# RomanJuranek/librectify

Hardware: AMD Instinct MI355X
Metric: Mpix/s end-to-end (detect+VP) on 4K frames, batch call of 64 frames, 5 in flight (higher is better)
Workload: dtype f32

## Files before the change

librectify_amd/csrc/common.h:

```cpp
#pragma once
#include <hip/hip_runtime.h>

#include <cstdint>
#include <string>

#include "../../include/librectify_amd.h"

namespace lramd {

constexpr float kEps = 1e-6f;
constexpr int kMaxModels = 4;
constexpr int kMaxPeelModels = 5;
constexpr float kInlierDeg = 2.0f;
constexpr float kGarbageDeg = 4.0f;
constexpr int kRansacMaxIter = 10000;
constexpr int kEdgeKernelSize = 2;
constexpr float kEdgeKernelSigma = 1.0f;
constexpr int kSeedDist = 2;
constexpr float kSeedRatio = 0.95f;
constexpr float kTraceTolerance = 0.25f;
constexpr float kLineMaxErr = 2.0f;
constexpr float kLineMinLength = 5.f;
constexpr int kComponentMinSize = 5;
constexpr int kBins = 8;
// ... 138 lines not shown
    BinTrig trig;
    uint32_t* label;
    int32_t* seed_size;
    int32_t* queue;
    const uint4* seed_rec;
};
struct FloodProgress {
    int enqueued = 0;
    bool use_big = false;
    int win_growth = 2;
    bool sizes_known = false;
    uint32_t max_flood = 0;
};
constexpr int kFloodCtrlWords = 56;
int flood_enqueue(const FloodBuffers& B, const FloodFrame& F, FloodProgress* P, uint32_t* h_ctrl, hipStream_t s);
int flood_finish(const FloodBuffers& B, const FloodFrame& F, FloodProgress* P, uint32_t* h_ctrl, int* rounds_out,
                 uint32_t* tiers_out ,
                 bool* extra, hipStream_t s);

size_t fit_temp_bytes(size_t max_pixels, uint32_t max_segments);
struct HugeSort {
    uint32_t* tab = nullptr;
    uint32_t* list = nullptr;
    uint32_t* jobs = nullptr;
    uint32_t max = 0;
};
int launch_component_offsets(const int32_t* seed_size, const uint32_t* d_n_seeds, uint32_t seed_cap, int min_size,
                             uint32_t* comp_rank, uint32_t* comp_seed, uint32_t* comp_off,
                             uint32_t* totals , uint32_t* large_list, uint32_t large_cap,
                             uint32_t* n_large, void* temp, size_t temp_bytes, uint32_t frame_tag, uint32_t* cursor, const HugeSort& hs,
                             hipStream_t s);
int launch_component_scatter(const uint32_t* label, size_t npix, const uint32_t* comp_rank, const uint32_t* comp_off,
                             uint32_t* cursor, uint32_t* px, const HugeSort& hs, uint32_t* n_large, bool with_huge, hipStream_t s);
int launch_component_sort(const uint32_t* px_in, uint32_t* px_out, const uint32_t* comp_off, const uint32_t* d_n_comp,
                          uint32_t comp_cap, const uint32_t* large_list, uint32_t large_cap, const uint32_t* n_large,
                          uint32_t* scratch, const uint32_t* cursor, const HugeSort& hs, bool with_huge, hipStream_t s);
int launch_fit(const uint32_t* px_sorted, const uint32_t* px_unsorted, const uint32_t* comp_off, const uint32_t* comp_seed, const uint32_t* d_n_comp,
               uint32_t comp_cap, const int32_t* seed_bin, const float* dx, const float* dy, int w, BinTrig trig,
               float* scratch_w, LineSegment* out, const uint32_t* cursor, const HugeSort& hs, const uint32_t* n_large, bool with_huge,
               hipStream_t s);

struct PencilSoA {
    const float* ax;
    const float* ay;
    const float* dx;
    const float* dy;
    const float* len;
    const float* hx;
    const float* hy;
    const float* hz;
};
constexpr int kRansacBestSlots = 32;
int launch_ransac_score(PencilSoA m, uint32_t n, float tol, float degeneracy_tol, uint32_t n_iter, uint64_t seed,
                        uint32_t round, unsigned long long* best_slots, uint32_t* host_best, hipStream_t s);
int launch_ransac_score_dev(PencilSoA m, const uint32_t* gctl, int max_models, float tol, float degeneracy_tol,
                            uint32_t n_iter, uint64_t seed, unsigned long long* best_slots, hipStream_t s);

struct PencilTable {
    float* ax;
    float* ay;
    float* dx;
    float* dy;
    float* len;
    float* hx;
    float* hy;
    float* hz;
    uint32_t* orig;
    PencilSoA soa() const { return PencilSoA{ax, ay, dx, dy, len, hx, hy, hz}; }
};
enum {
    kGcLines = 0,
    kGcRemaining = 1,
    kGcRound = 2,
// ... 30 lines not shown
```

librectify_amd/csrc/frame.hip:

```cpp
#include "host.h"

#include <cstdio>
#include <cstdlib>
#include <cstring>

namespace lramd {


namespace {

uint32_t round_up(uint32_t v, uint32_t m) { return (v + m - 1) / m * m; }

uint32_t initial_seed_cap(size_t npix) {
    return (uint32_t)std::min<size_t>(npix, std::max<size_t>(round_up((uint32_t)(npix / 32), 1024), 4096));
}

uint32_t line_cap_for(const lr_context* c) {
    return (uint32_t)std::min<size_t>(c->seed_cap, c->ws.cap_pix / 6 + 16);
}


PencilTable table_of(lr_context* c, int which) {
    const size_t cl = c->cap_glines;
    float* b = c->d_tables + (size_t)which * 8 * cl;
// ... 151 lines not shown
}

int finish_flood(lr_context* c, bool* extra) {
    *extra = false;
    if (c->opt.flood_mode == 0) return 0;
    if (flood_finish(flood_buffers_for(c), flood_frame_for(c), &c->flood_prog, c->h_counts + 16, &c->flood_rounds,
                     c->flood_tiers, extra, c->stream))
        return 1;
    static const bool call_debug = std::getenv("LIBRECTIFY_CALL_DEBUG") != nullptr;
    if (call_debug)
        std::fprintf(stderr, "flood: %d rounds, %u walks in the second tier, %u of them long, hold-back phase %u (started with it: %d)\n",
                     c->flood_rounds, c->flood_tiers[0], c->flood_tiers[8], c->flood_tiers[3], (int)c->flood_hold_hint);
    c->flood_logbig_hint = c->flood_tiers[0] > 0;
    c->flood_calm_hint = c->flood_tiers[0] == 0 && c->flood_tiers[1] == 0 && c->flood_tiers[15] == 0;
    c->flood_big_hint = true;
    c->flood_hold_hint = c->flood_tiers[3] != 0 && c->flood_tiers[8] >= 16;
    constexpr uint32_t kStagedKeep = 64;
    c->flood_staged_hint = c->flood_tiers[14] != 0 && (!c->flood_staged_hint || c->flood_tiers[0] >= kStagedKeep);
    c->flood_staged_streak = c->flood_staged_hint ? c->flood_staged_streak + 1 : 0;
    if (c->flood_staged_streak >= 16) {
        c->flood_staged_hint = false;
        c->flood_staged_streak = 0;
    }
    if (c->flood_staged_hint) c->flood_hold_hint = false;

    c->flood_rounds_hint = std::max(std::max(c->flood_rounds + 2, 6), c->flood_rounds_hint - 1);
    c->flood_rounds_last = c->flood_rounds;
    return 0;
}

int enqueue_fit(lr_context* c) {
    const size_t npix = (size_t)c->w * c->h;
    const uint32_t comp_cap = line_cap_for(c);
    const bool with_huge = !(c->opt.flood_mode != 0 && c->flood_prog.sizes_known && c->flood_prog.max_flood <= (1u << 14));
    if (launch_component_offsets(c->ws.seed_size, c->d_counts + kCntSeeds, c->seed_cap, kComponentMinSize, c->ws.comp_rank,
                                 c->ws.comp_seed, c->ws.comp_off, c->d_counts + kCntComp, c->ws.comp_large,
                                 (uint32_t)(c->ws.cap_pix / 64 + 16), c->d_counts + kCntLarge, c->ws.temp, c->ws.temp.cap(), ++c->fit_tag ? c->fit_tag : ++c->fit_tag, c->ws.cursor,
                                 with_huge ? c->ws.huge : HugeSort{}, c->stream))
        return 1;
    if (launch_component_scatter(c->ws.label, npix, c->ws.comp_rank, c->ws.comp_off, c->ws.cursor, c->ws.px_a, c->ws.huge, c->d_counts + kCntLarge, with_huge,
                                 c->stream))
        return 1;
    if (launch_component_sort(c->ws.px_a, c->ws.px_b, c->ws.comp_off, c->d_counts + kCntComp, comp_cap, c->ws.comp_large,
                              (uint32_t)(c->ws.cap_pix / 64 + 16), c->d_counts + kCntLarge, reinterpret_cast<uint32_t*>(c->ws.keys_b.get()),
                              c->ws.cursor, c->ws.huge, with_huge, c->stream))
        return 1;
    static const bool fit_debug = std::getenv("LIBRECTIFY_FIT_DEBUG") != nullptr;
    if (fit_debug) {
        uint32_t cnt[16];
        LR_HIP(hipStreamSynchronize(c->stream));
        LR_HIP(hipMemcpy(cnt, c->d_counts, sizeof(cnt), hipMemcpyDeviceToHost));
        std::fprintf(stderr, "fit: with_huge %d (sizes known %d, largest flood %u); seeds %u comps %u px %u; lists: %u of 65..1024 px, %u longer, %u huge in %u buckets; counter %u\n",
                     (int)with_huge, (int)c->flood_prog.sizes_known, c->flood_prog.max_flood, cnt[0], cnt[1], cnt[2], cnt[4], cnt[5], cnt[6], cnt[7], cnt[10]);
        const uint32_t nj = std::min<uint32_t>(cnt[7], 6);
        std::vector<uint32_t> jobs(4 * nj + 4);
        if (nj) LR_HIP(hipMemcpy(jobs.data(), c->ws.huge.jobs, nj * 16, hipMemcpyDeviceToHost));
        for (uint32_t j = 0; j < nj; ++j) std::fprintf(stderr, "   bucket job %u: start %u, %u px, table word %u\n", j, jobs[4 * j], jobs[4 * j + 1], jobs[4 * j + 2]);
    }
    if (launch_fit(c->ws.px_b, c->ws.px_a, c->ws.comp_off, c->ws.comp_seed, c->d_counts + kCntComp, comp_cap, c->ws.seed_bin, c->ws.dx, c->ws.dy, c->w,
                   c->trig, c->ws.scratch_w, c->ws.d_lines, c->ws.cursor, c->ws.huge, c->d_counts + kCntLarge, with_huge, c->stream))
        return 1;
    if (c->opt.timing_on) LR_HIP(hipEventRecord(c->ev[4], c->stream));
    return 0;
}

}

int enqueue_groups(lr_context* c, uint32_t line_cap, int max_models, float inlier_deg, float garbage_deg, int n_iter,
                   uint64_t seed, bool model_done, bool gather) {
    if (max_models > kMaxPeelModels) {
        set_error("estimate_line_pencils: max_models above " + std::to_string(kMaxPeelModels) + " (the reference uses 4, config.h:25)");
        return 1;
    }
    const float tol = cos_threshold(inlier_deg), garbage_tol = cos_threshold(garbage_deg);
    const PencilTable all = table_of(c, 0);
    PencilTable tab[2] = {table_of(c, 1), table_of(c, 2)};
    if (!model_done && launch_pencil_model(c->d_flines, c->d_gctl, c->d_gnorm, all, tab[0], line_cap, c->stream)) return 1;
    const float degeneracy_tol = 0.05f;
    for (int k = 0; k < max_models; ++k) {
        if (n_iter > 0 &&
            launch_ransac_score_dev(tab[k & 1].soa(), c->d_gctl, max_models, tol, degeneracy_tol, (uint32_t)n_iter, seed,
                                    c->d_best_slots, c->stream))
            return 1;
        const bool last = gather && k == max_models - 1;
        if (launch_peel(tab[k & 1], tab[(k + 1) & 1], all, c->d_best_slots, seed, tol, garbage_tol,
                        max_models, c->d_gctl, c->d_inl, c->d_flines, c->d_models, c->d_counts,
                        (uint32_t)std::min<size_t>(c->res_lines_cap, c->d_flines.cap()), last ? c->h_res.get() : nullptr, c->stream))
            return 1;
    }
    return 0;
}

namespace {
// ... 374 lines not shown
```

librectify_amd/csrc/kernels_fit.hip:

```cpp
#include <algorithm>
#include <cstring>

#include <atomic>

#include "common.h"

namespace lramd {
namespace {

constexpr uint32_t kNoComp = 0xFFFFFFFFu;

constexpr uint32_t kSortLds = 1024;
constexpr uint32_t kSortLdsBig = 16384;
constexpr uint32_t kHugeShift = 14;
constexpr uint32_t kHugeFlag = 0x80000000u;
constexpr int kOffPer = 8;
constexpr uint32_t kOffChunk = 256 * kOffPer;

__device__ __forceinline__ void chunk_counts(const int32_t* __restrict__ seed_size, uint32_t n_seeds, int min_size,
                                             uint32_t k0, int (&sz)[kOffPer], uint32_t& c, uint32_t& p) {
    c = p = 0;
#pragma unroll
    for (int j = 0; j < kOffPer; ++j) {
        sz[j] = (k0 + j < n_seeds) ? seed_size[k0 + j] : 0;
// ... 178 lines not shown
    if (nn > 0.0) {
        vr = vr / nn;
        vc = vc / nn;
    } else {
        vr = 1.0;
        vc = 0.0;
    }
    float fr = (float)vr, fc = (float)vc;
    if (fr < fc || (fr == fc && fr < 0.0f)) {
        fr = -fr;
        fc = -fc;
    }
    d_r = fr;
    d_c = fc;
}

template <int kThreads, class Keys>
__device__ __forceinline__ void bitonic_sort(Keys& key, uint32_t P) {
    for (uint32_t k = 2; k <= P; k <<= 1)
        for (uint32_t j = k >> 1; j > 0; j >>= 1) {
            for (uint32_t t = threadIdx.x; t < P / 2; t += kThreads) {
                const uint32_t i = 2 * t - (t & (j - 1));
                const uint32_t a = key[i], b = key[i + j];
                const bool up = (i & k) == 0;
                if ((a > b) == up) {
                    key[i] = b;
                    key[i + j] = a;
                }
            }
            __syncthreads();
        }
}

__global__ __launch_bounds__(256) void component_sort_large_kernel(const uint32_t* __restrict__ px_in,
                                                                   uint32_t* __restrict__ px_out,
                                                                   const uint32_t* __restrict__ comp_off,
                                                                   const uint32_t* __restrict__ large_list,
                                                                   const uint32_t* __restrict__ n_large) {
    __shared__ uint32_t s_key[kSortLds];
    const uint32_t n_list = n_large[0];
    for (uint32_t li = blockIdx.x; li < n_list; li += gridDim.x) {
        const uint32_t comp = large_list[li];
        const uint32_t off = comp_off[comp];
        const uint32_t n = comp_off[comp + 1] - off;
        uint32_t P = 128;
        while (P < n) P <<= 1;
        for (uint32_t i = threadIdx.x; i < P; i += 256) s_key[i] = i < n ? px_in[off + i] : 0xFFFFFFFFu;
        __syncthreads();
        bitonic_sort<256>(s_key, P);
        for (uint32_t i = threadIdx.x; i < n; i += 256) px_out[off + i] = s_key[i];
        __syncthreads();
    }
}

template <bool kGlobal>
__global__ __launch_bounds__(1024) void component_sort_big_kernel(const uint32_t* __restrict__ px_in,
                                                                  uint32_t* __restrict__ px_out,
                                                                  const uint32_t* __restrict__ comp_off,
                                                                  const uint32_t* __restrict__ large_list,
                                                                  uint32_t large_cap,
                                                                  const uint32_t* __restrict__ n_large,
                                                                  uint32_t* __restrict__ scratch,
                                                                  const uint32_t* __restrict__ cursor) {
    __shared__ uint32_t s_key[kGlobal ? 1 : kSortLdsBig];
    const uint32_t n_list = n_large[1];
    for (uint32_t li = blockIdx.x; li < n_list; li += gridDim.x) {
        const uint32_t comp = large_list[large_cap - 1u - li];
        const uint32_t off = comp_off[comp];
        const uint32_t n = comp_off[comp + 1] - off;
        if ((n > kSortLdsBig) != kGlobal) continue;
        if (kGlobal && cursor != nullptr && (cursor[comp] & kHugeFlag)) continue;
        uint32_t P = 2048;
        while (P < n) P <<= 1;
        if (!kGlobal) {
            for (uint32_t i = threadIdx.x; i < P; i += 1024) s_key[i] = i < n ? px_in[off + i] : 0xFFFFFFFFu;
            __syncthreads();
            bitonic_sort<1024>(s_key, P);
            for (uint32_t i = threadIdx.x; i < n; i += 1024) px_out[off + i] = s_key[i];
            __syncthreads();
        } else {
            for (uint32_t i = threadIdx.x; i < P; i += 1024) scratch[i] = i < n ? px_in[off + i] : 0xFFFFFFFFu;
            __syncthreads();
            bitonic_sort<1024>(scratch, P);
            for (uint32_t i = threadIdx.x; i < n; i += 1024) px_out[off + i] = scratch[i];
            __syncthreads();
        }
    }
}

__global__ __launch_bounds__(256) void huge_count_kernel(const uint32_t* __restrict__ label, size_t npix,
                                                         const uint32_t* __restrict__ comp_rank,
                                                         const uint32_t* __restrict__ comp_off,
                                                         const uint32_t* __restrict__ cursor, uint32_t* __restrict__ huge_tab,
                                                         uint32_t nb, const uint32_t* __restrict__ huge_list, uint32_t huge_max,
                                                         uint4* __restrict__ jobs, uint32_t* __restrict__ n_large) {
    const uint32_t n_huge = min(n_large[2], huge_max);
    if (n_huge == 0u) return;
    const int lane = threadIdx.x & 63;
    const size_t step = (size_t)gridDim.x * 256;
    const size_t n_pad = (npix + 255) / 256 * 256;
    for (size_t i = (size_t)blockIdx.x * 256 + threadIdx.x; i < n_pad; i += step) {
        const uint32_t l = i < npix ? label[i] : kLabelFree;
        const uint32_t r = l != kLabelFree ? comp_rank[l] : kNoComp;
        uint32_t hi = 0u;
        if (r != kNoComp && comp_off[r + 1u] - comp_off[r] > kSortLdsBig) hi = cursor[r];
        uint64_t todo = __ballot((hi & kHugeFlag) != 0u);
        while (todo != 0ull) {
            const int leader = __builtin_ctzll(todo);
            const uint32_t hl = (uint32_t)__builtin_amdgcn_readlane((int)hi, leader);
            const uint64_t same = __ballot(hi == hl) & todo;
            if (lane == leader) atomicAdd(&huge_tab[(size_t)(hl & ~kHugeFlag) * nb + (uint32_t)(i >> kHugeShift)], (uint32_t)__popcll(same));
            todo &= ~same;
        }
    }
    __shared__ uint32_t s_last;
    __syncthreads();
    if (threadIdx.x == 0) {
        __threadfence();
        s_last = atomicAdd(n_large + 6, 1u) == gridDim.x - 1u ? 1u : 0u;
// ... 14 lines not shown
            for (int off = 1; off < 64; off <<= 1) {
                const uint32_t t = (uint32_t)__shfl_up((int)inc, off);
                if (lane >= off) inc += t;
            }
            const uint32_t start = run + inc - cnt;
            if (cnt != 0u) {
                *e = start;
                jobs[atomicAdd(n_large + 3, 1u)] = make_uint4(start, cnt, h * nb + b, 0u);
            }
            run += (uint32_t)__shfl((int)inc, 63);
        }
    }
}

__global__ __launch_bounds__(1024) void huge_sort_kernel(const uint32_t* __restrict__ px_in, uint32_t* __restrict__ px_out,
                                                         const uint4* __restrict__ jobs, uint32_t* __restrict__ huge_tab,
                                                         const uint32_t* __restrict__ n_large) {
    __shared__ uint32_t s_key[kSortLdsBig];
    const uint32_t n_jobs = n_large[3];
    for (uint32_t j = blockIdx.x; j < n_jobs; j += gridDim.x) {
        const uint4 job = jobs[j];
        const uint32_t off = job.x, n = job.y;
        uint32_t P = 64;
        while (P < n) P <<= 1;
        for (uint32_t i = threadIdx.x; i < P; i += 1024) s_key[i] = i < n ? px_in[off + i] : 0xFFFFFFFFu;
        __syncthreads();
        bitonic_sort<1024>(s_key, P);
        for (uint32_t i = threadIdx.x; i < n; i += 1024) px_out[off + i] = s_key[i];
        if (threadIdx.x == 0) huge_tab[job.z] = 0u;
        __syncthreads();
    }
}

template <int kU>
__device__ __forceinline__ void fit_large(const uint32_t* __restrict__ px, uint32_t comp, uint32_t off, uint32_t n, float s, float c,
                                          uint32_t uw, const float* __restrict__ dx, const float* __restrict__ dy,
                                          float* __restrict__ scratch_w, LineSegment* __restrict__ out, int lane) {
    float acc = 0.f;
    for (uint32_t i0 = lane; i0 < n; i0 += 64u * kU) {
        uint32_t p[kU];
        float gx[kU], gy[kU];
#pragma unroll
        for (int u = 0; u < kU; ++u) {
            const uint32_t i = i0 + 64u * (uint32_t)u;
            p[u] = i < n ? px[off + i] : 0u;
        }
#pragma unroll
        for (int u = 0; u < kU; ++u) {
            gx[u] = dx[p[u]];
            gy[u] = dy[p[u]];
        }
#pragma unroll
        for (int u = 0; u < kU; ++u) {
            const uint32_t i = i0 + 64u * (uint32_t)u;
            if (i < n) {
                const float wv = directional(gx[u], gy[u], s, c);
                scratch_w[off + i] = wv;
                acc = acc + wv;
            }
        }
    }
    const float S = wave_tree(acc);

    float ar = 0.f, ac = 0.f;
    for (uint32_t i0 = lane; i0 < n; i0 += 64u * kU) {
        uint32_t p[kU];
// ... 42 lines not shown
    }
    const float cov_rr = wave_tree(crr), cov_rc = wave_tree(crc), cov_cc = wave_tree(ccc);

    float d_r, d_c;
    major_axis_2x2(cov_rr, cov_rc, cov_cc, d_r, d_c);
    const float n_r = -d_c, n_c = d_r;

    float t0 = INFINITY, t1 = -INFINITY, es = 0.f;
    for (uint32_t i0 = lane; i0 < n; i0 += 64u * kU) {
        uint32_t p[kU];
#pragma unroll
        for (int u = 0; u < kU; ++u) {
            const uint32_t i = i0 + 64u * (uint32_t)u;
            p[u] = i < n ? px[off + i] : 0u;
        }
#pragma unroll
        for (int u = 0; u < kU; ++u) {
            const uint32_t i = i0 + 64u * (uint32_t)u;
            if (i < n) {
                const float cr = (float)(p[u] / uw) - a_r, cc = (float)(p[u] % uw) - a_c;
                const float t = cr * d_r + cc * d_c;
                t0 = fminf(t0, t);
                t1 = fmaxf(t1, t);
                es = es + fabsf(cr * n_r + cc * n_c);
            }
        }
    }
#pragma unroll
    for (int o = 32; o >= 1; o >>= 1) {
        t0 = fminf(t0, __shfl_xor(t0, o));
        t1 = fmaxf(t1, __shfl_xor(t1, o));
    }
    const float esum = wave_tree(es);
    if (lane == 0) {
        LineSegment l;
        l.x1 = a_c + d_c * t0;
        l.y1 = a_r + d_r * t0;
        l.x2 = a_c + d_c * t1;
        l.y2 = a_r + d_r * t1;
        l.weight = S / (float)n;
        l.err = esum / (float)n;
        l.group_id = -1;
        out[comp] = l;
    }
}

__global__ __launch_bounds__(256) void fit_kernel(const uint32_t* __restrict__ px, const uint32_t* __restrict__ px_unsorted,
                                                  const uint32_t* __restrict__ comp_off,
                                                  const uint32_t* __restrict__ comp_seed, const uint32_t* __restrict__ n_comp_ptr,
                                                  const int32_t* __restrict__ seed_bin, const float* __restrict__ dx,
                                                  const float* __restrict__ dy, int w, BinTrig trig,
                                                  float* __restrict__ scratch_w, LineSegment* __restrict__ out,
                                                  const uint32_t* __restrict__ huge_cursor) {
    const int lane = threadIdx.x & 63;
    const uint32_t comp = blockIdx.x * 4 + (threadIdx.x >> 6);
    if (comp >= *n_comp_ptr) return;
    const uint32_t off = comp_off[comp];
    const uint32_t n = comp_off[comp + 1] - off;
    const int b = seed_bin[comp_seed[comp]];
    const float s = trig.st[b], c = trig.ct[b];
    const uint32_t uw = (uint32_t)w;

    if (n <= 64u) {
        const bool has = (uint32_t)lane < n;
        const uint32_t key = has ? px_unsorted[off + lane] : 0xFFFFFFFFu;
        uint32_t rank = 0;
#pragma unroll
        for (int j = 0; j < 64; ++j) rank += ((uint32_t)__builtin_amdgcn_readlane((int)key, j) < key) ? 1u : 0u;
        const uint32_t p_sorted = (uint32_t)__builtin_amdgcn_ds_permute((int)(min(rank, 63u) << 2), (int)key);
        const uint32_t p = has ? p_sorted : 0u;
        float wv = 0.f;
        if (has) wv = directional(dx[p], dy[p], s, c);
        float acc = 0.f;
        if (has) acc = acc + wv;
        const float S = wave_tree(acc);
        const float r = (float)(p / uw), cq = (float)(p % uw);
        const float wn = wv / S;
        float ar = 0.f, ac = 0.f;
        if (has) {
            ar = ar + wn * r;
            ac = ac + wn * cq;
        }
        const float a_r = wave_tree(ar), a_c = wave_tree(ac);
        const float cr = r - a_r, cc = cq - a_c;
        float crr = 0.f, crc = 0.f, ccc = 0.f;
        if (has) {
            const float t = cr * wn, u = cc * wn;
            crr = crr + t * cr;
            crc = crc + t * cc;
            ccc = ccc + u * cc;
        }
        const float cov_rr = wave_tree(crr), cov_rc = wave_tree(crc), cov_cc = wave_tree(ccc);
        float d_r, d_c;
        major_axis_2x2(cov_rr, cov_rc, cov_cc, d_r, d_c);
        const float n_r = -d_c, n_c = d_r;
        float t0 = INFINITY, t1 = -INFINITY, es = 0.f;
        if (has) {
            const float t = cr * d_r + cc * d_c;
            t0 = fminf(t0, t);
            t1 = fmaxf(t1, t);
            es = es + fabsf(cr * n_r + cc * n_c);
        }
#pragma unroll
        for (int o = 32; o >= 1; o >>= 1) {
            t0 = fminf(t0, __shfl_xor(t0, o));
            t1 = fmaxf(t1, __shfl_xor(t1, o));
        }
        const float esum = wave_tree(es);
        if (lane == 0) {
            LineSegment l;
            l.x1 = a_c + d_c * t0;
            l.y1 = a_r + d_r * t0;
            l.x2 = a_c + d_c * t1;
            l.y2 = a_r + d_r * t1;
            l.weight = S / (float)n;
            l.err = esum / (float)n;
            l.group_id = -1;
            out[comp] = l;
        }
        return;
    }

    if (huge_cursor != nullptr && n > kSortLdsBig && (huge_cursor[comp] & kHugeFlag) != 0u) return;
    fit_large<8>(px, comp, off, n, s, c, uw, dx, dy, scratch_w, out, lane);
}

__device__ __forceinline__ float huge_chunk_sum(float acc, const float* __restrict__ v, uint32_t cn, int lane) {
    for (uint32_t j0 = (uint32_t)lane; j0 < cn; j0 += 64u * 16u) {
        float t[16];
#pragma unroll
        for (int u = 0; u < 16; ++u) {
            const uint32_t j = j0 + 64u * (uint32_t)u;
            t[u] = j < cn ? v[j] : 0.f;
        }
#pragma unroll
        for (int u = 0; u < 16; ++u)
            if (j0 + 64u * (uint32_t)u < cn) acc = acc + t[u];
    }
    return acc;
}
constexpr int kHugeTerms = 24576;
constexpr size_t kHugeLdsBytes = (size_t)kHugeTerms * sizeof(float);
__global__ __launch_bounds__(1024) void fit_huge_kernel(const uint32_t* __restrict__ px, const uint32_t* __restrict__ comp_off,
                                                        const uint32_t* __restrict__ comp_seed, const uint32_t* __restrict__ huge_list,
                                                        const uint32_t* __restrict__ n_large, uint32_t huge_max,
                                                        const int32_t* __restrict__ seed_bin, const float* __restrict__ dx,
                                                        const float* __restrict__ dy, int w, BinTrig trig,
                                                        float* __restrict__ scratch_w, LineSegment* __restrict__ out) {
    extern __shared__ float s_terms[];
    __shared__ float s_res[3];
    __shared__ float s_mm[2][16];
    if (blockIdx.x >= min(n_large[2], huge_max)) return;
    const uint32_t comp = huge_list[blockIdx.x];
    const uint32_t off = comp_off[comp];
    const uint32_t n = comp_off[comp + 1] - off;
    const int b = seed_bin[comp_seed[comp]];
    const float s = trig.st[b], c = trig.ct[b];
    const uint32_t uw = (uint32_t)w;
    const int tid = (int)threadIdx.x, lane = tid & 63, wave = tid >> 6;

    float acc = 0.f;
    {
        constexpr uint32_t kC = 16384u;
        constexpr int kE = (int)(kC / 1024u);
        for (uint32_t c0 = 0; c0 < n; c0 += kC) {
            const uint32_t cn = min(kC, n - c0);
            uint32_t p[kE];
            float gx[kE], gy[kE];
#pragma unroll
            for (int e = 0; e < kE; ++e) {
                const uint32_t j = (uint32_t)tid + 1024u * (uint32_t)e;
                p[e] = j < cn ? px[off + c0 + j] : 0u;
            }
// ... 133 lines not shown
            if (wave == 0) acc = huge_chunk_sum(acc, s_terms, cn, lane);
            __syncthreads();
        }
    }
#pragma unroll
    for (int o = 32; o >= 1; o >>= 1) {
        t0 = fminf(t0, __shfl_xor(t0, o));
        t1 = fmaxf(t1, __shfl_xor(t1, o));
    }
    if (lane == 0) {
        s_mm[0][wave] = t0;
        s_mm[1][wave] = t1;
    }
    __syncthreads();
    if (wave != 0) return;
    const float esum = wave_tree(acc);
    if (lane == 0) {
        for (int i = 1; i < 16; ++i) {
            t0 = fminf(t0, s_mm[0][i]);
            t1 = fmaxf(t1, s_mm[1][i]);
        }
        LineSegment l;
        l.x1 = a_c + d_c * t0;
        l.y1 = a_r + d_r * t0;
        l.x2 = a_c + d_c * t1;
        l.y2 = a_r + d_r * t1;
        l.weight = S / (float)n;
        l.err = esum / (float)n;
        l.group_id = -1;
        out[comp] = l;
    }
}

}

size_t fit_temp_bytes(size_t max_pixels, uint32_t max_segments) {
    (void)max_segments;
    return (max_pixels / kOffChunk + 2) * 2 * sizeof(unsigned long long) + 256;
}

int launch_component_offsets(const int32_t* seed_size, const uint32_t* d_n_seeds, uint32_t seed_cap, int min_size,
                             uint32_t* comp_rank, uint32_t* comp_seed, uint32_t* comp_off, uint32_t* totals,
                             uint32_t* large_list, uint32_t large_cap, uint32_t* n_large, void* temp, size_t temp_bytes,
                             uint32_t frame_tag, uint32_t* cursor, const HugeSort& hs, hipStream_t s) {
    const uint32_t chunks = (seed_cap + kOffChunk - 1) / kOffChunk;
    if (chunks == 0 || temp_bytes < (size_t)chunks * 2 * sizeof(unsigned long long)) {
        set_error("launch_component_offsets: workspace too small");
        return 1;
    }
    hipLaunchKernelGGL(component_offsets_kernel, dim3(chunks), dim3(256), 0, s, seed_size, d_n_seeds, seed_cap, min_size,
                       static_cast<unsigned long long*>(temp), frame_tag, comp_rank, comp_seed, comp_off, totals, large_list, large_cap,
                       n_large, cursor, hs.list, hs.tab ? hs.max : 0u);
    LR_HIP(hipGetLastError());
    return 0;
}

int launch_component_scatter(const uint32_t* label, size_t npix, const uint32_t* comp_rank, const uint32_t* comp_off,
                             uint32_t* cursor, uint32_t* px, const HugeSort& hs, uint32_t* n_large, bool with_huge, hipStream_t s) {
    const uint32_t nb = (uint32_t)((npix + ((size_t)1 << kHugeShift) - 1) >> kHugeShift);
    const size_t want = (npix + 255) / 256;
    if (with_huge && hs.tab)
        hipLaunchKernelGGL(huge_count_kernel, dim3((unsigned)std::min<size_t>(want, 2048)), dim3(256), 0, s, label, npix, comp_rank, comp_off,
                           cursor, hs.tab, nb, hs.list, hs.max, reinterpret_cast<uint4*>(hs.jobs), n_large);
    const int blocks = (int)(want < 8192 ? want : 8192);
    hipLaunchKernelGGL(component_scatter_kernel, dim3(blocks > 0 ? blocks : 1), dim3(256), 0, s, label, npix, comp_rank,
                       comp_off, cursor, px, hs.tab, nb);
    LR_HIP(hipGetLastError());
    return 0;
}

int launch_component_sort(const uint32_t* px_in, uint32_t* px_out, const uint32_t* comp_off, const uint32_t* d_n_comp,
                          uint32_t comp_cap, const uint32_t* large_list, uint32_t large_cap, const uint32_t* n_large,
                          uint32_t* scratch, const uint32_t* cursor, const HugeSort& hs, bool with_huge, hipStream_t s) {
    if (comp_cap == 0) return 0;
    (void)d_n_comp;
    hipLaunchKernelGGL(component_sort_large_kernel, dim3(4096), dim3(256), 0, s, px_in, px_out, comp_off, large_list, n_large);
    hipLaunchKernelGGL(component_sort_big_kernel<false>, dim3(128), dim3(1024), 0, s, px_in, px_out, comp_off, large_list,
                       large_cap, n_large, scratch, cursor);
    if (with_huge && hs.tab) {
        hipLaunchKernelGGL(huge_sort_kernel, dim3(512), dim3(1024), 0, s, px_in, px_out, reinterpret_cast<const uint4*>(hs.jobs), hs.tab, n_large);
        hipLaunchKernelGGL(component_sort_big_kernel<true>, dim3(1), dim3(1024), 0, s, px_in, px_out, comp_off, large_list,
                           large_cap, n_large, scratch, cursor);
    }
    LR_HIP(hipGetLastError());
    return 0;
}

int launch_fit(const uint32_t* px_sorted, const uint32_t* px_unsorted, const uint32_t* comp_off, const uint32_t* comp_seed, const uint32_t* d_n_comp,
               uint32_t comp_cap, const int32_t* seed_bin, const float* dx, const float* dy, int w, BinTrig trig,
               float* scratch_w, LineSegment* out, const uint32_t* cursor, const HugeSort& hs, const uint32_t* n_large, bool with_huge,
               hipStream_t s) {
    if (comp_cap == 0) return 0;
    const bool huge = with_huge && hs.tab != nullptr && hs.max != 0u;
    if (huge) {
        static std::atomic<uint64_t> done_mask{0};
        int dev = 0;
        LR_HIP(hipGetDevice(&dev));
        const uint64_t bit = 1ull << (dev & 63);
        if (!(done_mask.load(std::memory_order_acquire) & bit)) {
            LR_HIP(hipFuncSetAttribute(reinterpret_cast<const void*>(fit_huge_kernel), hipFuncAttributeMaxDynamicSharedMemorySize, (int)kHugeLdsBytes));
            done_mask.fetch_or(bit, std::memory_order_release);
        }
        hipLaunchKernelGGL(fit_huge_kernel, dim3(hs.max), dim3(1024), kHugeLdsBytes, s, px_sorted, comp_off, comp_seed, hs.list, n_large, hs.max, seed_bin,
                           dx, dy, w, trig, scratch_w, out);
    }
    hipLaunchKernelGGL(fit_kernel, dim3((comp_cap + 3) / 4), dim3(256), 0, s, px_sorted, px_unsorted, comp_off, comp_seed, d_n_comp,
                       seed_bin, dx, dy, w, trig, scratch_w, out, huge ? cursor : nullptr);
    LR_HIP(hipGetLastError());
    return 0;
}

}
```

Measured before the change: 10640.

## Fuse mid and big component sorts into the fit kernels using LDS

Removes the separate sort kernels for mid-size and big components. Each fit block now sorts a component's pixels in LDS (a bitonic sort that finishes small strides with wave barriers) and fits the line straight from LDS, with a new fit_big_kernel that uses dynamic LDS. This cuts kernel launches and the global round-trip of sorted pixel lists. In exchange, fit_kernel uses more LDS per block, which may lower occupancy, and the grid grows by a fixed number of extra mid-size groups.

Measured after the change: 10720 (median of 6 runs). Within noise of the previous version (+0.8%).

```diff
diff --git a/librectify_amd/csrc/common.h b/librectify_amd/csrc/common.h
--- a/librectify_amd/csrc/common.h
+++ b/librectify_amd/csrc/common.h
@@ -194,13 +194,12 @@
                              hipStream_t s);
 int launch_component_scatter(const uint32_t* label, size_t npix, const uint32_t* comp_rank, const uint32_t* comp_off,
                              uint32_t* cursor, uint32_t* px, const HugeSort& hs, uint32_t* n_large, bool with_huge, hipStream_t s);
-int launch_component_sort(const uint32_t* px_in, uint32_t* px_out, const uint32_t* comp_off, const uint32_t* d_n_comp,
-                          uint32_t comp_cap, const uint32_t* large_list, uint32_t large_cap, const uint32_t* n_large,
-                          uint32_t* scratch, const uint32_t* cursor, const HugeSort& hs, bool with_huge, hipStream_t s);
+int launch_huge_sort(const uint32_t* px_in, uint32_t* px_out, const uint32_t* comp_off, const uint32_t* large_list, uint32_t large_cap,
+                     const uint32_t* n_large, uint32_t* scratch, const uint32_t* cursor, const HugeSort& hs, hipStream_t s);
 int launch_fit(const uint32_t* px_sorted, const uint32_t* px_unsorted, const uint32_t* comp_off, const uint32_t* comp_seed, const uint32_t* d_n_comp,
-               uint32_t comp_cap, const int32_t* seed_bin, const float* dx, const float* dy, int w, BinTrig trig,
-               float* scratch_w, LineSegment* out, const uint32_t* cursor, const HugeSort& hs, const uint32_t* n_large, bool with_huge,
-               hipStream_t s);
+               uint32_t comp_cap, const uint32_t* large_list, uint32_t large_cap, const int32_t* seed_bin, const float* dx, const float* dy,
+               int w, BinTrig trig, float* scratch_w, LineSegment* out, const uint32_t* cursor, const HugeSort& hs, const uint32_t* n_large,
+               bool with_huge, hipStream_t s);
 
 struct PencilSoA {
     const float* ax;
diff --git a/librectify_amd/csrc/frame.hip b/librectify_amd/csrc/frame.hip
--- a/librectify_amd/csrc/frame.hip
+++ b/librectify_amd/csrc/frame.hip
@@ -207,18 +207,18 @@
 int enqueue_fit(lr_context* c) {
     const size_t npix = (size_t)c->w * c->h;
     const uint32_t comp_cap = line_cap_for(c);
+    const uint32_t large_cap = (uint32_t)(c->ws.cap_pix / 64 + 16);
     const bool with_huge = !(c->opt.flood_mode != 0 && c->flood_prog.sizes_known && c->flood_prog.max_flood <= (1u << 14));
     if (launch_component_offsets(c->ws.seed_size, c->d_counts + kCntSeeds, c->seed_cap, kComponentMinSize, c->ws.comp_rank,
                                  c->ws.comp_seed, c->ws.comp_off, c->d_counts + kCntComp, c->ws.comp_large,
-                                 (uint32_t)(c->ws.cap_pix / 64 + 16), c->d_counts + kCntLarge, c->ws.temp, c->ws.temp.cap(), ++c->fit_tag ? c->fit_tag : ++c->fit_tag, c->ws.cursor,
+                                 large_cap, c->d_counts + kCntLarge, c->ws.temp, c->ws.temp.cap(), ++c->fit_tag ? c->fit_tag : ++c->fit_tag, c->ws.cursor,
                                  with_huge ? c->ws.huge : HugeSort{}, c->stream))
         return 1;
     if (launch_component_scatter(c->ws.label, npix, c->ws.comp_rank, c->ws.comp_off, c->ws.cursor, c->ws.px_a, c->ws.huge, c->d_counts + kCntLarge, with_huge,
                                  c->stream))
         return 1;
-    if (launch_component_sort(c->ws.px_a, c->ws.px_b, c->ws.comp_off, c->d_counts + kCntComp, comp_cap, c->ws.comp_large,
-                              (uint32_t)(c->ws.cap_pix / 64 + 16), c->d_counts + kCntLarge, reinterpret_cast<uint32_t*>(c->ws.keys_b.get()),
-                              c->ws.cursor, c->ws.huge, with_huge, c->stream))
+    if (with_huge && launch_huge_sort(c->ws.px_a, c->ws.px_b, c->ws.comp_off, c->ws.comp_large, large_cap, c->d_counts + kCntLarge,
+                                      reinterpret_cast<uint32_t*>(c->ws.keys_b.get()), c->ws.cursor, c->ws.huge, c->stream))
         return 1;
     static const bool fit_debug = std::getenv("LIBRECTIFY_FIT_DEBUG") != nullptr;
     if (fit_debug) {
@@ -232,8 +232,9 @@
         if (nj) LR_HIP(hipMemcpy(jobs.data(), c->ws.huge.jobs, nj * 16, hipMemcpyDeviceToHost));
         for (uint32_t j = 0; j < nj; ++j) std::fprintf(stderr, "   bucket job %u: start %u, %u px, table word %u\n", j, jobs[4 * j], jobs[4 * j + 1], jobs[4 * j + 2]);
     }
-    if (launch_fit(c->ws.px_b, c->ws.px_a, c->ws.comp_off, c->ws.comp_seed, c->d_counts + kCntComp, comp_cap, c->ws.seed_bin, c->ws.dx, c->ws.dy, c->w,
-                   c->trig, c->ws.scratch_w, c->ws.d_lines, c->ws.cursor, c->ws.huge, c->d_counts + kCntLarge, with_huge, c->stream))
+    if (launch_fit(c->ws.px_b, c->ws.px_a, c->ws.comp_off, c->ws.comp_seed, c->d_counts + kCntComp, comp_cap, c->ws.comp_large, large_cap, c->ws.seed_bin,
+                   c->ws.dx, c->ws.dy, c->w, c->trig, c->ws.scratch_w, c->ws.d_lines, c->ws.cursor, c->ws.huge, c->d_counts + kCntLarge, with_huge,
+                   c->stream))
         return 1;
     if (c->opt.timing_on) LR_HIP(hipEventRecord(c->ev[4], c->stream));
     return 0;
diff --git a/librectify_amd/csrc/kernels_fit.hip b/librectify_amd/csrc/kernels_fit.hip
--- a/librectify_amd/csrc/kernels_fit.hip
+++ b/librectify_amd/csrc/kernels_fit.hip
@@ -234,28 +234,38 @@
         }
 }
 
-__global__ __launch_bounds__(256) void component_sort_large_kernel(const uint32_t* __restrict__ px_in,
-                                                                   uint32_t* __restrict__ px_out,
-                                                                   const uint32_t* __restrict__ comp_off,
-                                                                   const uint32_t* __restrict__ large_list,
-                                                                   const uint32_t* __restrict__ n_large) {
-    __shared__ uint32_t s_key[kSortLds];
-    const uint32_t n_list = n_large[0];
-    for (uint32_t li = blockIdx.x; li < n_list; li += gridDim.x) {
-        const uint32_t comp = large_list[li];
-        const uint32_t off = comp_off[comp];
-        const uint32_t n = comp_off[comp + 1] - off;
-        uint32_t P = 128;
-        while (P < n) P <<= 1;
-        for (uint32_t i = threadIdx.x; i < P; i += 256) s_key[i] = i < n ? px_in[off + i] : 0xFFFFFFFFu;
-        __syncthreads();
-        bitonic_sort<256>(s_key, P);
-        for (uint32_t i = threadIdx.x; i < n; i += 256) px_out[off + i] = s_key[i];
-        __syncthreads();
-    }
-}
-
-template <bool kGlobal>
+template <int kThreads>
+__device__ __forceinline__ void bitonic_sort_lds(uint32_t* key, uint32_t P) {
+    static_assert(kThreads % 64 == 0, "a trip's pairs are whole wavefronts'");
+    for (uint32_t k = 2; k <= P; k <<= 1) {
+        uint32_t j = k >> 1;
+        for (; j > 64; j >>= 1) {
+            for (uint32_t t = threadIdx.x; t < P / 2; t += kThreads) {
+                const uint32_t i = 2 * t - (t & (j - 1));
+                const uint32_t a = key[i], b = key[i + j];
+                const bool up = (i & k) == 0;
+                if ((a > b) == up) {
+                    key[i] = b;
+                    key[i + j] = a;
+                }
+            }
+            __syncthreads();
+        }
+        for (uint32_t t = threadIdx.x; t < P / 2; t += kThreads)
+            for (uint32_t jj = j; jj > 0; jj >>= 1) {
+                const uint32_t i = 2 * t - (t & (jj - 1));
+                const uint32_t a = key[i], b = key[i + jj];
+                const bool up = (i & k) == 0;
+                if ((a > b) == up) {
+                    key[i] = b;
+                    key[i + jj] = a;
+                }
+                __builtin_amdgcn_wave_barrier();
+            }
+        if (k >= 128) __syncthreads();
+    }
+}
+
 __global__ __launch_bounds__(1024) void component_sort_big_kernel(const uint32_t* __restrict__ px_in,
                                                                   uint32_t* __restrict__ px_out,
                                                                   const uint32_t* __restrict__ comp_off,
@@ -264,29 +274,20 @@
                                                                   const uint32_t* __restrict__ n_large,
                                                                   uint32_t* __restrict__ scratch,
                                                                   const uint32_t* __restrict__ cursor) {
-    __shared__ uint32_t s_key[kGlobal ? 1 : kSortLdsBig];
     const uint32_t n_list = n_large[1];
     for (uint32_t li = blockIdx.x; li < n_list; li += gridDim.x) {
         const uint32_t comp = large_list[large_cap - 1u - li];
         const uint32_t off = comp_off[comp];
         const uint32_t n = comp_off[comp + 1] - off;
-        if ((n > kSortLdsBig) != kGlobal) continue;
-        if (kGlobal && cursor != nullptr && (cursor[comp] & kHugeFlag)) continue;
+        if (n <= kSortLdsBig) continue;
+        if (cursor != nullptr && (cursor[comp] & kHugeFlag)) continue;
         uint32_t P = 2048;
         while (P < n) P <<= 1;
-        if (!kGlobal) {
-            for (uint32_t i = threadIdx.x; i < P; i += 1024) s_key[i] = i < n ? px_in[off + i] : 0xFFFFFFFFu;
-            __syncthreads();
-            bitonic_sort<1024>(s_key, P);
-            for (uint32_t i = threadIdx.x; i < n; i += 1024) px_out[off + i] = s_key[i];
-            __syncthreads();
-        } else {
-            for (uint32_t i = threadIdx.x; i < P; i += 1024) scratch[i] = i < n ? px_in[off + i] : 0xFFFFFFFFu;
-            __syncthreads();
-            bitonic_sort<1024>(scratch, P);
-            for (uint32_t i = threadIdx.x; i < n; i += 1024) px_out[off + i] = scratch[i];
-            __syncthreads();
-        }
+        for (uint32_t i = threadIdx.x; i < P; i += 1024) scratch[i] = i < n ? px_in[off + i] : 0xFFFFFFFFu;
+        __syncthreads();
+        bitonic_sort<1024>(scratch, P);
+        for (uint32_t i = threadIdx.x; i < n; i += 1024) px_out[off + i] = scratch[i];
+        __syncthreads();
     }
 }
 
@@ -367,6 +368,34 @@
     }
 }
 
+__device__ __forceinline__ float huge_chunk_sum(float acc, const float* __restrict__ v, uint32_t cn, int lane) {
+    for (uint32_t j0 = (uint32_t)lane; j0 < cn; j0 += 64u * 16u) {
+        float t[16];
+#pragma unroll
+        for (int u = 0; u < 16; ++u) {
+            const uint32_t j = j0 + 64u * (uint32_t)u;
+            t[u] = j < cn ? v[j] : 0.f;
+        }
+#pragma unroll
+        for (int u = 0; u < 16; ++u)
+            if (j0 + 64u * (uint32_t)u < cn) acc = acc + t[u];
+    }
+    return acc;
+}
+
+__device__ __forceinline__ void store_segment(LineSegment* __restrict__ out, uint32_t comp, uint32_t n, float S, float a_r, float a_c,
+                                              float d_r, float d_c, float t0, float t1, float esum) {
+    LineSegment l;
+    l.x1 = a_c + d_c * t0;
+    l.y1 = a_r + d_r * t0;
+    l.x2 = a_c + d_c * t1;
+    l.y2 = a_r + d_r * t1;
+    l.weight = S / (float)n;
+    l.err = esum / (float)n;
+    l.group_id = -1;
+    out[comp] = l;
+}
+
 template <int kU>
 __device__ __forceinline__ void fit_large(const uint32_t* __restrict__ px, uint32_t comp, uint32_t off, uint32_t n, float s, float c,
                                           uint32_t uw, const float* __restrict__ dx, const float* __restrict__ dy,
@@ -475,36 +504,155 @@
         t1 = fmaxf(t1, __shfl_xor(t1, o));
     }
     const float esum = wave_tree(es);
-    if (lane == 0) {
-        LineSegment l;
-        l.x1 = a_c + d_c * t0;
-        l.y1 = a_r + d_r * t0;
-        l.x2 = a_c + d_c * t1;
-        l.y2 = a_r + d_r * t1;
-        l.weight = S / (float)n;
-        l.err = esum / (float)n;
-        l.group_id = -1;
-        out[comp] = l;
-    }
-}
-
-__global__ __launch_bounds__(256) void fit_kernel(const uint32_t* __restrict__ px, const uint32_t* __restrict__ px_unsorted,
-                                                  const uint32_t* __restrict__ comp_off,
+    if (lane == 0) store_segment(out, comp, n, S, a_r, a_c, d_r, d_c, t0, t1, esum);
+}
+
+template <int kU>
+__device__ __forceinline__ void fit_lds(const uint32_t* s_r, const float* s_c, float* s_w, uint32_t comp, uint32_t n,
+                                        LineSegment* __restrict__ out, int lane) {
+    const float S = wave_tree(huge_chunk_sum(0.f, s_w, n, lane));
+
+    float ar = 0.f, ac = 0.f;
+    for (uint32_t i0 = lane; i0 < n; i0 += 64u * kU) {
+        float r[kU], cq[kU], wq[kU];
+#pragma unroll
+        for (int u = 0; u < kU; ++u) {
+            const uint32_t i = i0 + 64u * (uint32_t)u;
+            r[u] = i < n ? __uint_as_float(s_r[i]) : 0.f;
+            cq[u] = i < n ? s_c[i] : 0.f;
+            wq[u] = i < n ? s_w[i] : 0.f;
+        }
+#pragma unroll
+        for (int u = 0; u < kU; ++u) {
+            const uint32_t i = i0 + 64u * (uint32_t)u;
+            if (i < n) {
+                const float wn = wq[u] / S;
+                s_w[i] = wn;
+                ar = ar + wn * r[u];
+                ac = ac + wn * cq[u];
+            }
+        }
+    }
+    const float a_r = wave_tree(ar), a_c = wave_tree(ac);
+
+    float crr = 0.f, crc = 0.f, ccc = 0.f;
+    for (uint32_t i0 = lane; i0 < n; i0 += 64u * kU) {
+        float r[kU], cq[kU], wq[kU];
+#pragma unroll
+        for (int u = 0; u < kU; ++u) {
+            const uint32_t i = i0 + 64u * (uint32_t)u;
+            r[u] = i < n ? __uint_as_float(s_r[i]) : 0.f;
+            cq[u] = i < n ? s_c[i] : 0.f;
+            wq[u] = i < n ? s_w[i] : 0.f;
+        }
+#pragma unroll
+        for (int u = 0; u < kU; ++u) {
+            if (i0 + 64u * (uint32_t)u < n) {
+                const float cr = r[u] - a_r, cc = cq[u] - a_c;
+                const float wn = wq[u];
+                const float t = cr * wn, u2 = cc * wn;
+                crr = crr + t * cr;
+                crc = crc + t * cc;
+                ccc = ccc + u2 * cc;
+            }
+        }
+    }
+    const float cov_rr = wave_tree(crr), cov_rc = wave_tree(crc), cov_cc = wave_tree(ccc);
+
+    float d_r, d_c;
+    major_axis_2x2(cov_rr, cov_rc, cov_cc, d_r, d_c);
+    const float n_r = -d_c, n_c = d_r;
+
+    float t0 = INFINITY, t1 = -INFINITY, es = 0.f;
+    for (uint32_t i0 = lane; i0 < n; i0 += 64u * kU) {
+        float r[kU], cq[kU];
+#pragma unroll
+        for (int u = 0; u < kU; ++u) {
+            const uint32_t i = i0 + 64u * (uint32_t)u;
+            r[u] = i < n ? __uint_as_float(s_r[i]) : 0.f;
+            cq[u] = i < n ? s_c[i] : 0.f;
+        }
+#pragma unroll
+        for (int u = 0; u < kU; ++u) {
+            if (i0 + 64u * (uint32_t)u < n) {
+                const float cr = r[u] - a_r, cc = cq[u] - a_c;
+                const float t = cr * d_r + cc * d_c;
+                t0 = fminf(t0, t);
+                t1 = fmaxf(t1, t);
+                es = es + fabsf(cr * n_r + cc * n_c);
+            }
+        }
+    }
+#pragma unroll
+    for (int o = 32; o >= 1; o >>= 1) {
+        t0 = fminf(t0, __shfl_xor(t0, o));
+        t1 = fmaxf(t1, __shfl_xor(t1, o));
+    }
+    const float esum = wave_tree(es);
+    if (lane == 0) store_segment(out, comp, n, S, a_r, a_c, d_r, d_c, t0, t1, esum);
+}
+
+__global__ __launch_bounds__(256) void fit_kernel(const uint32_t* __restrict__ px_unsorted, const uint32_t* __restrict__ comp_off,
                                                   const uint32_t* __restrict__ comp_seed, const uint32_t* __restrict__ n_comp_ptr,
-                                                  const int32_t* __restrict__ seed_bin, const float* __restrict__ dx,
-                                                  const float* __restrict__ dy, int w, BinTrig trig,
-                                                  float* __restrict__ scratch_w, LineSegment* __restrict__ out,
-                                                  const uint32_t* __restrict__ huge_cursor) {
+                                                  const uint32_t* __restrict__ large_list, const uint32_t* __restrict__ n_large,
+                                                  uint32_t mid_groups, const int32_t* __restrict__ seed_bin,
+                                                  const float* __restrict__ dx, const float* __restrict__ dy, int w, BinTrig trig,
+                                                  LineSegment* __restrict__ out) {
+    __shared__ uint32_t s_key[kSortLds];
+    __shared__ float s_col[kSortLds], s_wt[kSortLds];
     const int lane = threadIdx.x & 63;
-    const uint32_t comp = blockIdx.x * 4 + (threadIdx.x >> 6);
+    const uint32_t uw = (uint32_t)w;
+
+    if (blockIdx.x < mid_groups) {
+        const uint32_t n_list = n_large[0];
+        for (uint32_t li = blockIdx.x; li < n_list; li += mid_groups) {
+            const uint32_t comp = large_list[li];
+            const uint32_t off = comp_off[comp];
+            const uint32_t n = comp_off[comp + 1] - off;
+            const int b = seed_bin[comp_seed[comp]];
+            const float s = trig.st[b], c = trig.ct[b];
+            uint32_t P = 128;
+            while (P < n) P <<= 1;
+            for (uint32_t i = threadIdx.x; i < P; i += 256) s_key[i] = i < n ? px_unsorted[off + i] : 0xFFFFFFFFu;
+            __syncthreads();
+            bitonic_sort_lds<256>(s_key, P);
+            constexpr int kE = (int)(kSortLds / 256u);
+            uint32_t p[kE];
+            float gx[kE], gy[kE];
+#pragma unroll
+            for (int e = 0; e < kE; ++e) {
+                const uint32_t i = threadIdx.x + 256u * (uint32_t)e;
+                p[e] = i < n ? s_key[i] : 0u;
+            }
+#pragma unroll
+            for (int e = 0; e < kE; ++e) {
+                gx[e] = dx[p[e]];
+                gy[e] = dy[p[e]];
+            }
+#pragma unroll
+            for (int e = 0; e < kE; ++e) {
+                const uint32_t i = threadIdx.x + 256u * (uint32_t)e;
+                if (i < n) {
+                    s_wt[i] = directional(gx[e], gy[e], s, c);
+                    s_key[i] = __float_as_uint((float)(p[e] / uw));
+                    s_col[i] = (float)(p[e] % uw);
+                }
+            }
+            __syncthreads();
+            if (threadIdx.x < 64u) fit_lds<4>(s_key, s_col, s_wt, comp, n, out, lane);
+            __syncthreads();
+        }
+        return;
+    }
+
+    const uint32_t comp = (blockIdx.x - mid_groups) * 4 + (threadIdx.x >> 6);
     if (comp >= *n_comp_ptr) return;
     const uint32_t off = comp_off[comp];
     const uint32_t n = comp_off[comp + 1] - off;
+    if (n > 64u) return;
     const int b = seed_bin[comp_seed[comp]];
     const float s = trig.st[b], c = trig.ct[b];
-    const uint32_t uw = (uint32_t)w;
-
-    if (n <= 64u) {
+    {
         const bool has = (uint32_t)lane < n;
         const uint32_t key = has ? px_unsorted[off + lane] : 0xFFFFFFFFu;
         uint32_t rank = 0;
@@ -550,38 +698,10 @@
             t1 = fmaxf(t1, __shfl_xor(t1, o));
         }
         const float esum = wave_tree(es);
-        if (lane == 0) {
-            LineSegment l;
-            l.x1 = a_c + d_c * t0;
-            l.y1 = a_r + d_r * t0;
-            l.x2 = a_c + d_c * t1;
-            l.y2 = a_r + d_r * t1;
-            l.weight = S / (float)n;
-            l.err = esum / (float)n;
-            l.group_id = -1;
-            out[comp] = l;
-        }
-        return;
-    }
-
-    if (huge_cursor != nullptr && n > kSortLdsBig && (huge_cursor[comp] & kHugeFlag) != 0u) return;
-    fit_large<8>(px, comp, off, n, s, c, uw, dx, dy, scratch_w, out, lane);
-}
-
-__device__ __forceinline__ float huge_chunk_sum(float acc, const float* __restrict__ v, uint32_t cn, int lane) {
-    for (uint32_t j0 = (uint32_t)lane; j0 < cn; j0 += 64u * 16u) {
-        float t[16];
-#pragma unroll
-        for (int u = 0; u < 16; ++u) {
-            const uint32_t j = j0 + 64u * (uint32_t)u;
-            t[u] = j < cn ? v[j] : 0.f;
-        }
-#pragma unroll
-        for (int u = 0; u < 16; ++u)
-            if (j0 + 64u * (uint32_t)u < cn) acc = acc + t[u];
-    }
-    return acc;
-}
+        if (lane == 0) store_segment(out, comp, n, S, a_r, a_c, d_r, d_c, t0, t1, esum);
+    }
+}
+
 constexpr int kHugeTerms = 24576;
 constexpr size_t kHugeLdsBytes = (size_t)kHugeTerms * sizeof(float);
 __global__ __launch_bounds__(1024) void fit_huge_kernel(const uint32_t* __restrict__ px, const uint32_t* __restrict__ comp_off,
@@ -781,6 +901,171 @@
     }
 }
 
+constexpr uint32_t kBigTerms = 6144;
+constexpr size_t kBigLdsBytes = (size_t)(2u * kSortLdsBig + kBigTerms) * sizeof(uint32_t);
+__global__ __launch_bounds__(1024) void fit_big_kernel(const uint32_t* __restrict__ px_unsorted, const uint32_t* __restrict__ px_sorted,
+                                                       const uint32_t* __restrict__ comp_off, const uint32_t* __restrict__ comp_seed,
+                                                       const uint32_t* __restrict__ large_list, uint32_t large_cap,
+                                                       const uint32_t* __restrict__ n_large, const uint32_t* __restrict__ cursor,
+                                                       const int32_t* __restrict__ seed_bin, const float* __restrict__ dx,
+                                                       const float* __restrict__ dy, int w, BinTrig trig,
+                                                       float* __restrict__ scratch_w, LineSegment* __restrict__ out) {
+    extern __shared__ uint32_t s_big[];
+    __shared__ float s_res[3];
+    __shared__ float s_mm[2][16];
+    uint32_t* s_key = s_big;
+    float* s_w = reinterpret_cast<float*>(s_big + kSortLdsBig);
+    float* s_terms = reinterpret_cast<float*>(s_big + 2u * kSortLdsBig);
+    const uint32_t uw = (uint32_t)w;
+    const int tid = (int)threadIdx.x, lane = tid & 63, wave = tid >> 6;
+    const uint32_t n_list = n_large[1];
+    for (uint32_t li = blockIdx.x; li < n_list; li += gridDim.x) {
+        const uint32_t comp = large_list[large_cap - 1u - li];
+        const uint32_t off = comp_off[comp];
+        const uint32_t n = comp_off[comp + 1] - off;
+        const int b = seed_bin[comp_seed[comp]];
+        const float s = trig.st[b], c = trig.ct[b];
+        if (n > kSortLdsBig) {
+            if (px_sorted != nullptr && (cursor[comp] & kHugeFlag) == 0u && wave == 0)
+                fit_large<8>(px_sorted, comp, off, n, s, c, uw, dx, dy, scratch_w, out, lane);
+            continue;
+        }
+        uint32_t P = 2048;
+        while (P < n) P <<= 1;
+        for (uint32_t i = threadIdx.x; i < P; i += 1024) s_key[i] = i < n ? px_unsorted[off + i] : 0xFFFFFFFFu;
+        __syncthreads();
+        bitonic_sort_lds<1024>(s_key, P);
+
+        {
+            constexpr int kE = (int)(kSortLdsBig / 1024u);
+            uint32_t p[kE];
+            float gx[kE], gy[kE];
+#pragma unroll
+            for (int e = 0; e < kE; ++e) {
+                const uint32_t j = (uint32_t)tid + 1024u * (uint32_t)e;
+                p[e] = j < n ? s_key[j] : 0u;
+            }
+#pragma unroll
+            for (int e = 0; e < kE; ++e) {
+                gx[e] = dx[p[e]];
+                gy[e] = dy[p[e]];
+            }
+#pragma unroll
+            for (int e = 0; e < kE; ++e) {
+                const uint32_t j = (uint32_t)tid + 1024u * (uint32_t)e;
+                if (j < n) s_w[j] = directional(gx[e], gy[e], s, c);
+            }
+        }
+        __syncthreads();
+        if (wave == 0) {
+            const float t = wave_tree(huge_chunk_sum(0.f, s_w, n, lane));
+            if (lane == 0) s_res[0] = t;
+        }
+        __syncthreads();
+        const float S = s_res[0];
+        __syncthreads();
+
+        float acc = 0.f;
+        {
+            constexpr uint32_t kC = kBigTerms / 2;
+            constexpr int kE = (int)(kC / 1024u);
+            static_assert(kC % 1024u == 0u, "a chunk is a whole number of elements per thread");
+            for (uint32_t c0 = 0; c0 < n; c0 += kC) {
+                const uint32_t cn = min(kC, n - c0);
+#pragma unroll
+                for (int e = 0; e < kE; ++e) {
+                    const uint32_t j = (uint32_t)tid + 1024u * (uint32_t)e;
+                    if (j < cn) {
+                        const uint32_t q = s_key[c0 + j];
+                        const float r = (float)(q / uw), cc = (float)(q % uw);
+                        const float wn = s_w[c0 + j] / S;
+                        s_w[c0 + j] = wn;
+                        s_terms[j] = wn * r;
+                        s_terms[kC + j] = wn * cc;
+                    }
+                }
+                __syncthreads();
+                if (wave < 2) acc = huge_chunk_sum(acc, s_terms + (size_t)wave * kC, cn, lane);
+                __syncthreads();
+            }
+        }
+        if (wave < 2) {
+            const float t = wave_tree(acc);
+            if (lane == 0) s_res[wave] = t;
+        }
+        __syncthreads();
+        const float a_r = s_res[0], a_c = s_res[1];
+        __syncthreads();
+
+        acc = 0.f;
+        {
+            constexpr uint32_t kC = kBigTerms / 3;
+            constexpr int kE = (int)(kC / 1024u);
+            static_assert(kC % 1024u == 0u, "a chunk is a whole number of elements per thread");
+            for (uint32_t c0 = 0; c0 < n; c0 += kC) {
+                const uint32_t cn = min(kC, n - c0);
+#pragma unroll
+                for (int e = 0; e < kE; ++e) {
+                    const uint32_t j = (uint32_t)tid + 1024u * (uint32_t)e;
+                    if (j < cn) {
+                        const uint32_t q = s_key[c0 + j];
+                        const float cr = (float)(q / uw) - a_r, cc = (float)(q % uw) - a_c;
+                        const float wn = s_w[c0 + j];
+                        const float t = cr * wn, u2 = cc * wn;
+                        s_terms[j] = t * cr;
+                        s_terms[kC + j] = t * cc;
+                        s_terms[2u * kC + j] = u2 * cc;
+                    }
+                }
+                __syncthreads();
+                if (wave < 3) acc = huge_chunk_sum(acc, s_terms + (size_t)wave * kC, cn, lane);
+                __syncthreads();
+            }
+        }
+        if (wave < 3) {
+            const float t = wave_tree(acc);
+            if (lane == 0) s_res[wave] = t;
+        }
+        __syncthreads();
+        const float cov_rr = s_res[0], cov_rc = s_res[1], cov_cc = s_res[2];
+
+        float d_r, d_c;
+        major_axis_2x2(cov_rr, cov_rc, cov_cc, d_r, d_c);
+        const float n_r = -d_c, n_c = d_r;
+
+        float t0 = INFINITY, t1 = -INFINITY;
+        for (uint32_t j = (uint32_t)tid; j < n; j += 1024u) {
+            const uint32_t q = s_key[j];
+            const float cr = (float)(q / uw) - a_r, cc = (float)(q % uw) - a_c;
+            const float t = cr * d_r + cc * d_c;
+            t0 = fminf(t0, t);
+            t1 = fmaxf(t1, t);
+            s_w[j] = fabsf(cr * n_r + cc * n_c);
+        }
+#pragma unroll
+        for (int o = 32; o >= 1; o >>= 1) {
+            t0 = fminf(t0, __shfl_xor(t0, o));
+            t1 = fmaxf(t1, __shfl_xor(t1, o));
+        }
+        if (lane == 0) {
+            s_mm[0][wave] = t0;
+            s_mm[1][wave] = t1;
+        }
+        __syncthreads();
+        if (wave == 0) {
+            const float esum = wave_tree(huge_chunk_sum(0.f, s_w, n, lane));
+            if (lane == 0) {
+                for (int i = 1; i < 16; ++i) {
+                    t0 = fminf(t0, s_mm[0][i]);
+                    t1 = fmaxf(t1, s_mm[1][i]);
+                }
+                store_segment(out, comp, n, S, a_r, a_c, d_r, d_c, t0, t1, esum);
+            }
+        }
+        __syncthreads();
+    }
+}
+
 }
 
 size_t fit_temp_bytes(size_t max_pixels, uint32_t max_segments) {
@@ -818,43 +1103,52 @@
     return 0;
 }
 
-int launch_component_sort(const uint32_t* px_in, uint32_t* px_out, const uint32_t* comp_off, const uint32_t* d_n_comp,
-                          uint32_t comp_cap, const uint32_t* large_list, uint32_t large_cap, const uint32_t* n_large,
-                          uint32_t* scratch, const uint32_t* cursor, const HugeSort& hs, bool with_huge, hipStream_t s) {
-    if (comp_cap == 0) return 0;
-    (void)d_n_comp;
-    hipLaunchKernelGGL(component_sort_large_kernel, dim3(4096), dim3(256), 0, s, px_in, px_out, comp_off, large_list, n_large);
-    hipLaunchKernelGGL(component_sort_big_kernel<false>, dim3(128), dim3(1024), 0, s, px_in, px_out, comp_off, large_list,
-                       large_cap, n_large, scratch, cursor);
-    if (with_huge && hs.tab) {
-        hipLaunchKernelGGL(huge_sort_kernel, dim3(512), dim3(1024), 0, s, px_in, px_out, reinterpret_cast<const uint4*>(hs.jobs), hs.tab, n_large);
-        hipLaunchKernelGGL(component_sort_big_kernel<true>, dim3(1), dim3(1024), 0, s, px_in, px_out, comp_off, large_list,
-                           large_cap, n_large, scratch, cursor);
-    }
+int launch_huge_sort(const uint32_t* px_in, uint32_t* px_out, const uint32_t* comp_off, const uint32_t* large_list, uint32_t large_cap,
+                     const uint32_t* n_large, uint32_t* scratch, const uint32_t* cursor, const HugeSort& hs, hipStream_t s) {
+    if (!hs.tab) return 0;
+    hipLaunchKernelGGL(huge_sort_kernel, dim3(512), dim3(1024), 0, s, px_in, px_out, reinterpret_cast<const uint4*>(hs.jobs), hs.tab, n_large);
+    hipLaunchKernelGGL(component_sort_big_kernel, dim3(1), dim3(1024), 0, s, px_in, px_out, comp_off, large_list, large_cap, n_large,
+                       scratch, cursor);
     LR_HIP(hipGetLastError());
     return 0;
 }
 
+namespace {
+
+int allow_dynamic_lds(const void* kernel, size_t bytes, std::atomic<uint64_t>& done_mask) {
+    int dev = 0;
+    LR_HIP(hipGetDevice(&dev));
+    const uint64_t bit = 1ull << (dev & 63);
+    if (!(done_mask.load(std::memory_order_acquire) & bit)) {
+        LR_HIP(hipFuncSetAttribute(kernel, hipFuncAttributeMaxDynamicSharedMemorySize, (int)bytes));
+        done_mask.fetch_or(bit, std::memory_order_release);
+    }
+    return 0;
+}
+
+constexpr uint32_t kMidGroups = 4096;
+constexpr uint32_t kBigGroups = 64;
+
+}
+
 int launch_fit(const uint32_t* px_sorted, const uint32_t* px_unsorted, const uint32_t* comp_off, const uint32_t* comp_seed, const uint32_t* d_n_comp,
-               uint32_t comp_cap, const int32_t* seed_bin, const float* dx, const float* dy, int w, BinTrig trig,
-               float* scratch_w, LineSegment* out, const uint32_t* cursor, const HugeSort& hs, const uint32_t* n_large, bool with_huge,
-               hipStream_t s) {
+               uint32_t comp_cap, const uint32_t* large_list, uint32_t large_cap, const int32_t* seed_bin, const float* dx, const float* dy,
+               int w, BinTrig trig, float* scratch_w, LineSegment* out, const uint32_t* cursor, const HugeSort& hs, const uint32_t* n_large,
+               bool with_huge, hipStream_t s) {
     if (comp_cap == 0) return 0;
     const bool huge = with_huge && hs.tab != nullptr && hs.max != 0u;
     if (huge) {
         static std::atomic<uint64_t> done_mask{0};
-        int dev = 0;
-        LR_HIP(hipGetDevice(&dev));
-        const uint64_t bit = 1ull << (dev & 63);
-        if (!(done_mask.load(std::memory_order_acquire) & bit)) {
-            LR_HIP(hipFuncSetAttribute(reinterpret_cast<const void*>(fit_huge_kernel), hipFuncAttributeMaxDynamicSharedMemorySize, (int)kHugeLdsBytes));
-            done_mask.fetch_or(bit, std::memory_order_release);
-        }
+        if (allow_dynamic_lds(reinterpret_cast<const void*>(fit_huge_kernel), kHugeLdsBytes, done_mask)) return 1;
         hipLaunchKernelGGL(fit_huge_kernel, dim3(hs.max), dim3(1024), kHugeLdsBytes, s, px_sorted, comp_off, comp_seed, hs.list, n_large, hs.max, seed_bin,
                            dx, dy, w, trig, scratch_w, out);
     }
-    hipLaunchKernelGGL(fit_kernel, dim3((comp_cap + 3) / 4), dim3(256), 0, s, px_sorted, px_unsorted, comp_off, comp_seed, d_n_comp,
-                       seed_bin, dx, dy, w, trig, scratch_w, out, huge ? cursor : nullptr);
+    static std::atomic<uint64_t> big_done_mask{0};
+    if (allow_dynamic_lds(reinterpret_cast<const void*>(fit_big_kernel), kBigLdsBytes, big_done_mask)) return 1;
+    hipLaunchKernelGGL(fit_big_kernel, dim3(kBigGroups), dim3(1024), kBigLdsBytes, s, px_unsorted, huge ? px_sorted : nullptr, comp_off, comp_seed,
+                       large_list, large_cap, n_large, cursor, seed_bin, dx, dy, w, trig, scratch_w, out);
+    hipLaunchKernelGGL(fit_kernel, dim3(kMidGroups + (comp_cap + 3) / 4), dim3(256), 0, s, px_unsorted, comp_off, comp_seed, d_n_comp, large_list, n_large,
+                       kMidGroups, seed_bin, dx, dy, w, trig, out);
     LR_HIP(hipGetLastError());
     return 0;
 }
```
